# lache/word2vec

Hardware: AMD Instinct MI355X
Metric: trained words/sec, dim=300 SGNS (per-GPU replica, RCCL all-reduce of the replicas' updates for N>1) (higher is better)
Workload: dtype fp32; 1 GPU; sg_ns neg5 d300 w5 subsample 0.0001 min_count 5; synthetic Zipf(s=1) over 1000000 ranks standing in for 1B-Word (configs[2]); 1000-token sentences; vocab_size=740391, global_batch=50000000, parallelism=dp1, hot_rows=-2, private_rows=-1, flush_centers=0, max_waves=0, context_rows=-1, context_flush=0, env_knobs=

## Files before the change

### include/w2v_dev.h

```cpp
#ifndef W2V_DEV_H
#define W2V_DEV_H

#include <stdint.h>

#ifdef __cplusplus
extern "C" {
#endif

#define W2V_OK 0
#define W2V_ERR_ARG 1
#define W2V_ERR_HIP 2
#define W2V_ERR_STATE 3
#define W2V_ERR_UNSUPPORTED 4
#define W2V_ERR_DIVERGED 5
#define W2V_ERR_COMM 6

#define W2V_RNG_PHILOX 0
#define W2V_RNG_REPLAY 1

#define W2V_SCHED_PARALLEL 0
#define W2V_SCHED_SEQUENTIAL 1

#define W2V_UPDATE_PER_PAIR 0
#define W2V_UPDATE_SHARED_NEGATIVES 1
// ... 57 lines not shown
int w2v_dev_upload_corpus(w2v_dev* h, const int32_t* ids, int64_t n_tokens,
                          const int64_t* sent_offsets, int64_t n_sentences,
                          int64_t train_words);
int w2v_dev_share_corpus(w2v_dev* h, w2v_dev* src);
int w2v_dev_upload_replay(w2v_dev* h, const uint32_t* stream, int64_t n,
                          const int64_t* stream_offsets, int64_t n_offsets);

int w2v_dev_set_progress(w2v_dev* h, int64_t current_words);
int w2v_dev_get_progress(w2v_dev* h, int64_t* current_words);
int w2v_dev_set_progress_async(w2v_dev* h, int64_t current_words);
int w2v_dev_set_train_words(w2v_dev* h, int64_t train_words);

int w2v_dev_train_epoch(w2v_dev* h, int32_t epoch, const int64_t* order, w2v_dev_stats* stats);
int w2v_dev_train_epoch_async(w2v_dev* h, int32_t epoch, const int64_t* order_dev);
int w2v_dev_train_sentences_async(w2v_dev* h, int32_t epoch, const int64_t* order_dev, int64_t count);
int w2v_dev_set_order(w2v_dev* h, const int64_t* order, int64_t n);
int w2v_dev_train_slice_async(w2v_dev* h, int32_t epoch, int64_t first, int64_t count);
int w2v_dev_synchronize(w2v_dev* h);
int w2v_dev_read_stats(w2v_dev* h, w2v_dev_stats* stats);
int w2v_dev_reset_stats(w2v_dev* h);

#define W2V_HOT_AUTO (-2)
int w2v_dev_set_hot_rows(w2v_dev* h, int64_t hot_rows);
int w2v_dev_set_hot_auto(w2v_dev* h, float tau_rows, float tau_nodes);
int w2v_dev_hot_tau(w2v_dev* h, float* tau_rows, float* tau_nodes);
int w2v_dev_policy(w2v_dev* h, int64_t* hot_rows, int64_t* hot_nodes, int32_t* private_rows, int32_t* context_rows);
int w2v_dev_flush_policy(w2v_dev* h, int32_t* flush_centers, int32_t* context_flush);
int w2v_dev_row_update_rates(w2v_dev* h, int32_t which, double* out, int64_t n);
int w2v_dev_set_private_rows(w2v_dev* h, int32_t n);
int w2v_dev_set_private_rate(w2v_dev* h, float mu);
int w2v_dev_private_rate_used(w2v_dev* h, float* mu);
int w2v_dev_wave_cap_used(w2v_dev* h, int64_t* waves);
int w2v_dev_deep_used(w2v_dev* h, int32_t* deep);
typedef struct w2v_launch_plan {
  int32_t shared;
  int32_t deep;
  int64_t grid;
  int32_t threads;
  int32_t wpb;
  int64_t lds_bytes;
  int64_t wave_cap;
  int32_t hot_wc;
  int32_t hot_s;
  int64_t hot_atomic;
  int64_t hot_nodes;
  int32_t priv_lo;
  int32_t priv_n;
  int32_t ctx_n;
  float priv_avg;
  int32_t flush_every;
  int32_t ctx_flush_every;
  int32_t nseg;
  int32_t seg_len;
  double private_rate;
  double tau_rows;
  double hs_hot_avg;
  int64_t wide_scratch;
  int64_t n_hot_sc;
  float priv_sc[128];
  float ctx_sc[64];
} w2v_launch_plan;
int w2v_dev_launch_plan(w2v_dev* h, w2v_launch_plan* out, float* hot_sc, int64_t hot_sc_cap);
int w2v_dev_set_replica_count(w2v_dev* h, int32_t n);
int w2v_dev_replica_count(w2v_dev* h, int32_t* n);
int w2v_dev_set_private_sync(w2v_dev* h, int32_t flush_centers, float average_over);
int w2v_dev_set_context_private(w2v_dev* h, int32_t rows, int32_t flush_centers);
// ... 66 lines not shown
```

### word2vec_amd/_native.py

```python
from __future__ import annotations

import ctypes as C
import os
from pathlib import Path

LIB_DIR = Path(__file__).resolve().parent / "lib"
DEV_LIB = LIB_DIR / "libw2v_hip.so"

W2V_OK = 0
W2V_ERR_ARG = 1
W2V_ERR_HIP = 2
W2V_ERR_STATE = 3
W2V_ERR_UNSUPPORTED = 4
W2V_ERR_DIVERGED = 5
W2V_ERR_COMM = 6
W2V_GROUP_ID_BYTES = 128
W2V_GROUP_SUM = 0
W2V_GROUP_AVERAGE = 1
W2V_GROUP_ROW_AVERAGE = 2
W2V_GROUP_ADAPTIVE = 3
W2V_GROUP_SPLIT = 4
W2V_GROUP_SATURATION = 5
W2V_RNG_PHILOX = 0
W2V_RNG_REPLAY = 1
# ... 78 lines not shown
    "w2v_dev_upload_vocab": (C.c_int, [_P, _I64, _P, _P, _P, _P, _P]),
    "w2v_dev_upload_table": (C.c_int, [_P, _P, _I64]),
    "w2v_dev_upload_model": (C.c_int, [_P, _P, _P, _P]),
    "w2v_dev_download_model": (C.c_int, [_P, _P, _P, _P]),
    "w2v_dev_upload_rows": (C.c_int, [_P, _I32, _P, _I64, _P]),
    "w2v_dev_download_rows": (C.c_int, [_P, _I32, _P, _I64, _P]),
    "w2v_dev_bind_model": (C.c_int, [_P, _P, _P, _P, _I64]),
    "w2v_dev_row_pitch": (C.c_int, [_P, C.POINTER(_I64)]),
    "w2v_dev_model_layout": (C.c_int, [_P, C.POINTER(_P), C.POINTER(_P), C.POINTER(_P), C.POINTER(_I64)]),
    "w2v_dev_upload_corpus": (C.c_int, [_P, _P, _I64, _P, _I64, _I64]),
    "w2v_dev_share_corpus": (C.c_int, [_P, _P]),
    "w2v_dev_upload_replay": (C.c_int, [_P, _P, _I64, _P, _I64]),
    "w2v_dev_set_progress": (C.c_int, [_P, _I64]),
    "w2v_dev_get_progress": (C.c_int, [_P, C.POINTER(_I64)]),
    "w2v_dev_set_progress_async": (C.c_int, [_P, _I64]),
    "w2v_dev_set_train_words": (C.c_int, [_P, _I64]),
    "w2v_dev_train_epoch": (C.c_int, [_P, _I32, _P, C.POINTER(DevStats)]),
    "w2v_dev_train_epoch_async": (C.c_int, [_P, _I32, _P]),
    "w2v_dev_train_sentences_async": (C.c_int, [_P, _I32, _P, _I64]),
    "w2v_dev_synchronize": (C.c_int, [_P]),
    "w2v_dev_set_order": (C.c_int, [_P, _P, _I64]),
    "w2v_dev_train_slice_async": (C.c_int, [_P, _I32, _I64, _I64]),
    "w2v_dev_read_stats": (C.c_int, [_P, C.POINTER(DevStats)]),
    "w2v_dev_reset_stats": (C.c_int, [_P]),
    "w2v_dev_set_fixed_alpha": (C.c_int, [_P, _F]),
    "w2v_dev_set_hot_rows": (C.c_int, [_P, _I64]),
    "w2v_dev_set_hot_auto": (C.c_int, [_P, _F, _F]),
    "w2v_dev_policy": (C.c_int, [_P, C.POINTER(_I64), C.POINTER(_I64), C.POINTER(_I32), C.POINTER(_I32)]),
    "w2v_dev_flush_policy": (C.c_int, [_P, C.POINTER(_I32), C.POINTER(_I32)]),
    "w2v_dev_hot_tau": (C.c_int, [_P, C.POINTER(_F), C.POINTER(_F)]),
    "w2v_dev_private_rate_used": (C.c_int, [_P, C.POINTER(_F)]),
    "w2v_dev_wave_cap_used": (C.c_int, [_P, C.POINTER(_I64)]),
    "w2v_dev_deep_used": (C.c_int, [_P, C.POINTER(_I32)]),
    "w2v_dev_launch_plan": (C.c_int, [_P, C.POINTER(LaunchPlan), C.POINTER(C.c_float), _I64]),
    "w2v_dev_set_replica_count": (C.c_int, [_P, _I32]),
    "w2v_dev_model_max_diff": (C.c_int, [_P, _P, C.POINTER(_F)]),
    "w2v_dev_replica_count": (C.c_int, [_P, C.POINTER(_I32)]),
    "w2v_dev_set_private_rows": (C.c_int, [_P, _I32]),
    "w2v_dev_set_private_rate": (C.c_int, [_P, _F]),
    "w2v_dev_set_private_sync": (C.c_int, [_P, _I32, _F]),
    "w2v_dev_set_context_private": (C.c_int, [_P, _I32, _I32]),
    "w2v_dev_set_max_waves": (C.c_int, [_P, _I64]),
    "w2v_dev_set_update": (C.c_int, [_P, _I32]),
    "w2v_dev_apply_rows": (C.c_int, [_P, _P, _P, _I32, _P, _P, _F, _I32]),
    "w2v_dev_score_limits": (C.c_int, [C.POINTER(_I32)] * 3),
    "w2v_dev_set_score_item": (C.c_int, [_P, _I32]),
    "w2v_dev_score": (C.c_int, [_P, _P, _I64, _P, _I64, _U64, _P, _P, C.POINTER(ScoreSummary)]),
    "w2v_group_unique_id": (C.c_int, [_P]),
    "w2v_group_create": (C.c_int, [_P, _I32, _P, _I32, _I32, C.POINTER(_P)]),
    "w2v_group_destroy": (None, [_P]),
    "w2v_group_set_overlap": (C.c_int, [_P, _I32]),
    "w2v_group_set_mode": (C.c_int, [_P, _I32]),
    "w2v_group_set_split": (C.c_int, [_P, _I64, _F]),
    "w2v_group_set_saturation": (C.c_int, [_P, _I64, _F]),
    "w2v_group_row_divisors": (C.c_int, [_P, _I32, C.POINTER(_F), _I64]),
    "w2v_dev_row_update_rates": (C.c_int, [_P, _I32, C.POINTER(C.c_double), _I64]),
    "w2v_group_split_rows": (C.c_int, [_P, C.POINTER(_I64)]),
    "w2v_group_average_async": (C.c_int, [_P]),
    "w2v_group_average_rows_async": (C.c_int, [_P, _I64]),
    "w2v_group_finish": (C.c_int, [_P]),
    "w2v_group_info": (C.c_int, [_P, C.POINTER(_I32), C.POINTER(_I32), C.POINTER(_I32), C.POINTER(_I64)]),
    "w2v_nn_limits": (C.c_int, [C.POINTER(_I32)] * 3),
    "w2v_nn_create": (C.c_int, [_I32, _P, _I64, _I32, C.POINTER(_P)]),
    "w2v_nn_attach": (C.c_int, [_P, _I32, C.POINTER(_P)]),
    "w2v_nn_refresh": (C.c_int, [_P]),
    "w2v_nn_destroy": (None, [_P]),
# ... 73 lines not shown
```

### word2vec_amd/csrc/device/w2v_dev.hip

```cpp
#include <hip/hip_runtime.h>

#include <cstdio>
#include <cstdlib>
#include <algorithm>
#include <cmath>
#include <cstdint>
#include <cstring>
#include <memory>
#include <string>
#include <utility>
#include <vector>

#include "w2v_dev.h"
#include "w2v_dev_internal.hpp"
#include "w2v_kernels.hpp"
#include "w2v_launch.hpp"
#include "w2v_policy.hpp"
#include "w2v_score.hpp"
#include "w2v_shared.hpp"

namespace w2v {

__global__ void expand_table_kernel(const int64_t* bounds, int64_t V, uint32_t* table, int64_t n) {
  const int64_t stride = (int64_t)gridDim.x * blockDim.x;
// ... 76 lines not shown
  w2v::DevBuf<int32_t> points;
  w2v::DevBuf<int64_t> coff;
  int64_t n_codes = 0;
  std::shared_ptr<CorpusBuf> corpus;
  int64_t n_tok = 0, n_sent = 0, train_words = 0;
  int64_t max_len = 0;
  w2v::DevBuf<int64_t> order;
  int64_t n_order = 0;
  w2v::DevBuf<uint32_t> replay;
  w2v::DevBuf<int64_t> replay_off;
  int64_t n_replay_off = 0;
  w2v::DevBuf<unsigned long long> counters;
  w2v::DevBuf<unsigned int> work;
  w2v::DevBuf<float> scratch_f;
  w2v::DevBuf<uint8_t> scratch_codes;
  w2v::DevBuf<int32_t> wide_scratch;
  w2v::DevBuf<float> xfer_f;
  float fixed_alpha = 0.0f;
  int32_t rng = W2V_RNG_PHILOX;
  uint64_t seed = 0;
  int32_t sched = W2V_SCHED_PARALLEL;
  int32_t update = W2V_UPDATE_PER_PAIR;
  int n_cu = 256;
  bool model_ready = false, vocab_ready = false, corpus_ready = false;
  std::vector<float> keep_h;
  std::vector<int32_t> leaf_node;
  std::vector<int32_t> node_parent;
  std::vector<int64_t> tok_count;
  uint64_t data_version = 0;
  uint64_t stats_version = ~0ull;
  w2v::RowStats stats;
  int32_t replicas = 1;
  w2v::LaunchPlan last_plan;
  std::vector<float> hot_sc_h;
  w2v::DevBuf<float> hot_sc_d;
  int32_t score_item = 0;
  w2v::DevBuf<int32_t> score_ids;
  w2v::DevBuf<int64_t> score_soff, score_item_off, score_part_targets, score_targets;
  w2v::DevBuf<double> score_part_ll, score_ll;
  w2v::DevBuf<uint32_t> score_part_nonfinite;
  w2v::DevBuf<unsigned long long> score_ctr;

  ~w2v_dev() {
    (void)hipSetDevice(device);
    if (stream) (void)hipStreamSynchronize(stream);
    if (own_stream && stream) (void)hipStreamDestroy(stream);
  }
  void drop_model() {
    W_own.reset(), C_own.reset(), S_own.reset();
    W = C = S = nullptr;
  }
};

namespace w2v {
int set_error(int code, const std::string& msg) { return fail(code, msg); }
DevInfo dev_info(const w2v_dev* h) { return DevInfo{h->device, h->stream, h->V, h->cfg.word_dim}; }
void set_replicas(w2v_dev* h, int32_t n) { h->replicas = n < 1 ? 1 : n; }
}

static const w2v::RowStats& stats_of(w2v_dev* h) {
  if (h->stats_version != h->data_version) {
    h->stats_version = h->data_version;
    w2v::row_stats(h->stats, h->V, h->tok_count, h->keep_h, h->leaf_node, h->node_parent);
  }
  return h->stats;
}
// ... 8 lines not shown
  for (int64_t c : h->tok_count) N += (double)c;
  const double q = N > 0.0 ? st.kept_tokens / N : 0.0;
  const double win1 = (double)h->cfg.window + 1.0, neg = (double)h->cfg.negative;
  const bool cbow = h->cfg.cbow != 0;
  if (k == 2) {
    if (!st.has_nodes(V)) return false;
    out.resize((size_t)(V - 1));
    for (int64_t j = 0; j < V - 1; ++j) out[(size_t)j] = q * st.node_rate(j, cbow, win1);
    return true;
  }
  out.resize((size_t)V);
  for (int64_t r = 0; r < V; ++r) {
    const double f = st.f[(size_t)r], fk = st.fk[(size_t)r];
    double m;
    if (k == 0) m = cbow ? (neg > 0 ? fk + neg * st.u(r) : 0.0) : fk;
    else m = cbow ? win1 * f : win1 * (f + neg * st.u(r));
    out[(size_t)r] = q * m;
  }
  return true;
}
}

namespace {

using KernelFn = w2v::KernelFn;

const w2v::NvKernels& kernels_for_need(int need) {
  for (const w2v::NvKernels& k : w2v::kNvKernels)
    if (k.nv >= need) return k;
  return *(std::end(w2v::kNvKernels) - 1);
}
int pick_nv(int d) { return kernels_for_need((d + w2v::kWave - 1) / w2v::kWave).nv; }

KernelFn kernel_for(const w2v_dev* h) {
  const bool wd = 2 * h->cfg.window + 1 > w2v::kWave;
  return kernels_for_need(h->nv).pick_train(h->cfg.cbow != 0, h->cfg.hs != 0, h->cfg.negative > 0,
                                            h->rng == W2V_RNG_REPLAY, wd);
}
KernelFn kernel_deep_for(const w2v_dev* h) { return kernels_for_need(h->nv).pick_train_deep(h->cfg.cbow != 0); }
w2v::ApplyFn apply_for(const w2v_dev* h) { return kernels_for_need(h->nv).pick_apply(); }

int set_device(w2v_dev* h) {
  W2V_HIP_TRY(hipSetDevice(h->device));
  return W2V_OK;
}

int install_corpus(w2v_dev* h, std::shared_ptr<CorpusBuf> c, int64_t n_tok, int64_t n_sent, int64_t max_len,
                   int64_t train_words, std::vector<int64_t> hist) {
  w2v::DevBuf<int64_t> order;
  if (int rc = order.alloc((size_t)(n_sent > 0 ? n_sent : 1))) return rc;
  h->corpus = std::move(c);
  h->order = std::move(order);
  h->n_tok = n_tok;
  h->n_sent = n_sent;
  h->n_order = 0;
  h->max_len = max_len;
  h->train_words = train_words;
  h->tok_count = std::move(hist);
  ++h->data_version;
  h->corpus_ready = true;
  return W2V_OK;
}

int init_device(w2v_dev* h) {
  W2V_HIP_TRY(hipSetDevice(h->device));
  W2V_HIP_TRY(hipStreamCreateWithFlags(&h->stream, hipStreamNonBlocking));
  h->own_stream = true;
  if (int rc = h->counters.alloc(8)) return rc;
  W2V_HIP_TRY(hipMemset(h->counters.get(), 0, 8 * sizeof(unsigned long long)));
  if (int rc = h->work.alloc(1)) return rc;
// ... 633 lines not shown
  }
  return W2V_OK;
}

static int launch_train(w2v_dev* h, int32_t epoch, const int64_t* order_dev, int64_t count) {
  w2v::Range range_("w2v launch");
  if (!h->vocab_ready || !h->corpus_ready) return fail(W2V_ERR_STATE, "upload vocab and corpus first");
  if (!h->model_ready) return fail(W2V_ERR_STATE, "upload the model first");
  if (h->cfg.negative > 0 && !h->table.get()) return fail(W2V_ERR_STATE, "no unigram table on the device");
  if (h->rng == W2V_RNG_REPLAY) {
    if (!h->replay.get()) return fail(W2V_ERR_STATE, "replay mode without a replay stream");
    if ((int64_t)(epoch + 1) * h->n_sent > h->n_replay_off)
      return fail(W2V_ERR_ARG, "replay offsets do not cover this epoch");
  }
  if (epoch < 0) return fail(W2V_ERR_ARG, "epoch must be >= 0");
  KernelFn sn_fn = nullptr;
  int sn_waves = 0;
  if (h->update == W2V_UPDATE_SHARED_NEGATIVES) {
    if (int rc = check_shared_negatives(h, true)) return rc;
    const int occ = h->knobs.sn_occ;
    if ((double)h->V * (double)h->pitch * sizeof(float) >= 4294967296.0)
      return fail(W2V_ERR_UNSUPPORTED, "shared negatives: W / C must be < 4 GiB each (32-bit buffer offsets)");
    if (!(sn_fn = w2v::pick_shared_neg(h->pitch, occ, &sn_waves)))
      return fail(W2V_ERR_UNSUPPORTED, "shared negatives: row pitch must be 64 * {1..8,10,12,14,16} floats");
  }
  if (count == 0) return W2V_OK;
  if (set_device(h)) return W2V_ERR_HIP;
  w2v::TrainArgs a{};
  a.W = h->W; a.C = h->C; a.S = h->S;
  a.pitch = h->pitch; a.dim = h->cfg.word_dim;
  a.window = h->cfg.window; a.negative = h->cfg.negative; a.cbow_mean = h->cfg.cbow_mean;
  a.iter = h->cfg.iter; a.init_alpha = h->cfg.init_alpha; a.min_alpha = h->cfg.min_alpha;
  a.train_words = (double)h->train_words;
  a.ids = h->corpus->ids.get(); a.soff = h->corpus->soff.get(); a.order = order_dev; a.n_sent = count; a.n_corpus = h->n_sent;
  a.keep = h->keep.get(); a.table = h->table.get(); a.table_size = h->cfg.table_size;
  a.codes = h->codes.get(); a.points = h->points.get(); a.coff = h->coff.get();
  a.replay = h->replay.get();
  a.replay_off = h->replay_off.get() ? h->replay_off.get() + (int64_t)epoch * h->n_sent : nullptr;
  a.words = h->counters.get();
  a.work = h->work.get();
  a.stats = h->counters.get() + 1;
  a.key0 = (uint32_t)h->seed; a.key1 = (uint32_t)(h->seed >> 32);
  a.epoch = (uint32_t)epoch;
  a.fixed_alpha = h->fixed_alpha;
  a.strict = h->sched == W2V_SCHED_SEQUENTIAL ? 1 : 0;
  W2V_HIP_TRY(hipMemsetAsync(h->work.get(), 0, sizeof(unsigned int), h->stream));
  const KernelFn occ_fn = sn_fn ? sn_fn : kernel_for(h), deep_fn = sn_fn ? sn_fn : kernel_deep_for(h);
  hipError_t occ_err = hipSuccess;
  auto occupancy = [&](w2v::OccKernel k, int threads, int64_t lds) {
    int per_cu = 0;
    const hipError_t e = hipOccupancyMaxActiveBlocksPerMultiprocessor(
        &per_cu, k == w2v::kOccTrainDeep ? deep_fn : occ_fn, threads, (size_t)lds);
    if (e != hipSuccess) occ_err = e;
    return per_cu;
  };
  w2v::LaunchPlan p = w2v::plan_launch(policy_input(h, count, sn_waves), occupancy);
  if (occ_err != hipSuccess)
    return fail(W2V_ERR_HIP, std::string("hipOccupancyMaxActiveBlocksPerMultiprocessor: ") + hipGetErrorString(occ_err));
  if (p.private_rate < 0.0) p.private_rate = h->last_plan.private_rate;
  if (p.tau_rows < 0.0) p.tau_rows = h->last_plan.tau_rows;
  if (p.hs_hot_avg < 0.0) p.hs_hot_avg = h->last_plan.hs_hot_avg;
  a.hot_wc = p.hot_wc; a.hot_s = p.hot_s; a.hot_atomic = p.hot_atomic;
  a.priv_lo = p.priv_lo; a.priv_n = p.priv_n; a.ctx_n = p.ctx_n; a.priv_avg = p.priv_avg;
  a.flush_every = p.flush_every; a.ctx_flush_every = p.ctx_flush_every;
  a.nseg = p.nseg; a.seg_len = p.seg_len;
  std::memcpy(a.priv_sc, p.priv_sc, sizeof(a.priv_sc));
  std::memcpy(a.ctx_sc, p.ctx_sc, sizeof(a.ctx_sc));
  if (!p.shared) {
    if (p.priv_n > 0) a.priv_M = h->cfg.hs ? h->S : (h->cfg.cbow ? h->W : h->C);
    if (p.ctx_n > 0) a.ctx_M = h->C;
  }
  if (int rc = launch_buffers(h, p, a)) return rc;
  const KernelFn fn = p.deep ? deep_fn : occ_fn;
  const dim3 grid((unsigned)p.grid), block((unsigned)p.threads);
  const size_t lds_bytes = (size_t)p.lds_bytes;
  h->last_plan = std::move(p);
  hipLaunchKernelGGL(fn, grid, block, lds_bytes, h->stream, a);
  W2V_HIP_TRY(hipGetLastError());
  return W2V_OK;
}

int w2v_dev_train_epoch(w2v_dev* h, int32_t epoch, const int64_t* order, w2v_dev_stats* st) {
  w2v::Range range_("w2v_dev_train_epoch");
  if (!h) return fail(W2V_ERR_ARG, "null handle");
  w2v_dev_stats before{};
  {
    int rc = w2v_dev_read_stats(h, &before);
    if (rc) return rc;
  }
  const int64_t* od = nullptr;
  if (order) {
    for (int64_t k = 0; k < h->n_sent; ++k)
      if (order[k] < 0 || order[k] >= h->n_sent) return fail(W2V_ERR_ARG, "order entry out of range");
    if (set_device(h)) return W2V_ERR_HIP;
    W2V_HIP_TRY(hipMemcpyAsync(h->order.get(), order, h->n_sent * sizeof(int64_t), hipMemcpyHostToDevice, h->stream));
    od = h->order.get();
    h->n_order = h->n_sent;
  }
  int rc = w2v_dev_train_epoch_async(h, epoch, od);
  if (rc) return rc;
  W2V_HIP_TRY(hipStreamSynchronize(h->stream));
  w2v_dev_stats after{};
  rc = w2v_dev_read_stats(h, &after);
  if (rc) return rc;
  if (st) {
    st->words += after.words - before.words;
    st->centers += after.centers - before.centers;
    st->contexts += after.contexts - before.contexts;
// ... 106 lines not shown
}

int w2v_dev_policy(w2v_dev* h, int64_t* hot_rows, int64_t* hot_nodes, int32_t* private_rows, int32_t* context_rows) {
  if (!h) return fail(W2V_ERR_ARG, "null handle");
  if (hot_rows) *hot_rows = h->last_plan.hot_rows;
  if (hot_nodes) *hot_nodes = h->last_plan.hot_nodes;
  if (private_rows) *private_rows = h->last_plan.priv_n;
  if (context_rows) *context_rows = h->last_plan.ctx_n;
  return W2V_OK;
}

int w2v_dev_hot_tau(w2v_dev* h, float* tau_rows, float* tau_nodes) {
  if (!h) return fail(W2V_ERR_ARG, "null handle");
  if (tau_rows) *tau_rows = (float)h->last_plan.tau_rows;
  if (tau_nodes) *tau_nodes = (float)h->set.hot_tau_nodes;
  return W2V_OK;
}

int w2v_dev_private_rate_used(w2v_dev* h, float* mu) {
  if (!h) return fail(W2V_ERR_ARG, "null handle");
  if (mu) *mu = (float)h->last_plan.private_rate;
  return W2V_OK;
}

int w2v_dev_wave_cap_used(w2v_dev* h, int64_t* waves) {
  if (!h) return fail(W2V_ERR_ARG, "null handle");
  if (waves) *waves = h->last_plan.wave_cap;
  return W2V_OK;
}

int w2v_dev_deep_used(w2v_dev* h, int32_t* deep) {
  if (!h || !deep) return fail(W2V_ERR_ARG, "null argument");
  *deep = h->last_plan.deep ? 1 : 0;
  return W2V_OK;
}

int w2v_dev_launch_plan(w2v_dev* h, w2v_launch_plan* out, float* hot_sc, int64_t hot_sc_cap) {
  if (!h || !out) return fail(W2V_ERR_ARG, "null argument");
  *out = h->last_plan;
  out->n_hot_sc = (int64_t)h->last_plan.hot_sc.size();
  if (hot_sc) std::copy_n(h->last_plan.hot_sc.begin(), std::min(hot_sc_cap, out->n_hot_sc), hot_sc);
  return W2V_OK;
}

int w2v_dev_set_replica_count(w2v_dev* h, int32_t n) {
  if (!h) return fail(W2V_ERR_ARG, "null handle");
  if (n < 1) return fail(W2V_ERR_ARG, "replica count must be >= 1");
  w2v::set_replicas(h, n);
  return W2V_OK;
}

int w2v_dev_replica_count(w2v_dev* h, int32_t* n) {
  if (!h || !n) return fail(W2V_ERR_ARG, "null argument");
  *n = h->replicas;
  return W2V_OK;
}

int w2v_dev_row_update_rates(w2v_dev* h, int32_t which, double* out, int64_t n) {
  if (!h || !out) return fail(W2V_ERR_ARG, "null argument");
  if (which < 0 || which > 2) return fail(W2V_ERR_ARG, "which must be 0 (W), 1 (C) or 2 (synapses1)");
  std::vector<double> rate;
  if (!w2v::row_update_rates(h, which, rate)) return fail(W2V_ERR_STATE, "no vocab / corpus statistics uploaded");
  if (n != (int64_t)rate.size()) return fail(W2V_ERR_ARG, "n must be the matrix's row count");
  std::copy(rate.begin(), rate.end(), out);
  return W2V_OK;
}
// ... 175 lines not shown
```

### word2vec_amd/csrc/device/w2v_inst.hip

```cpp
#include "w2v_kernels.hpp"
#include "w2v_launch.hpp"

#ifndef W2V_NV
#error "build with -DW2V_NV=<floats per lane>"
#endif

#define W2V_CAT2(a, b) a##b
#define W2V_CAT(a, b) W2V_CAT2(a, b)

namespace w2v {

constexpr int kMaxT = W2V_NV <= 16 ? 8 : 4;

KernelFn W2V_CAT(pick_train_nv, W2V_NV)(bool cbow, bool hs, bool ns, bool replay, bool wide) {
#define W2V_K(CB, H, N, R, WD) &train_epoch_kernel<W2V_NV, kMaxT, CB, H, N, R, WD>
#define W2V_KR(CB, H, N, WD) (replay ? W2V_K(CB, H, N, true, WD) : W2V_K(CB, H, N, false, WD))
#define W2V_KW(H, N) (wide ? W2V_KR(true, H, N, true) : W2V_KR(true, H, N, false))
  if (cbow) {
    if (hs && ns) return W2V_KW(true, true);
    if (hs) return W2V_KW(true, false);
    return W2V_KW(false, true);
  }
  if (hs && ns) return W2V_KR(false, true, true, false);
  if (hs) return W2V_KR(false, true, false, false);
  return W2V_KR(false, false, true, false);
#undef W2V_KW
#undef W2V_KR
#undef W2V_K
}

KernelFn W2V_CAT(pick_train_deep_nv, W2V_NV)(bool cbow) {
  constexpr int M = kDeepMaxT<W2V_NV>;
  return cbow ? &train_epoch_deep_kernel<W2V_NV, M, true, true, false, false, false>
              : &train_epoch_deep_kernel<W2V_NV, M, false, true, false, false, false>;
}

ApplyFn W2V_CAT(pick_apply_nv, W2V_NV)() { return &apply_rows_kernel<W2V_NV>; }

}
```

### word2vec_amd/csrc/device/w2v_kernels.hpp

```cpp
#pragma once
#include <hip/hip_runtime.h>
#include <stdint.h>

#include "w2v_limits.hpp"
#include "w2v_philox.hpp"
#include "w2v_rows.hpp"
#include "w2v_wave.hpp"

namespace w2v {


struct TrainArgs {
  float* W;
  float* C;
  float* S;
  int64_t pitch;
  int32_t dim;
  int32_t window;
  int32_t negative;
  int32_t cbow_mean;
  int32_t iter;
  float init_alpha;
  float min_alpha;
  double train_words;
// ... 5 lines not shown
  const float* keep;
  const uint32_t* table;
  int64_t table_size;
  const uint8_t* codes;
  const int32_t* points;
  const int64_t* coff;
  const uint32_t* replay;
  const int64_t* replay_off;
  unsigned long long* words;
  unsigned int* work;
  unsigned long long* stats;
  uint32_t key0, key1, epoch;
  float fixed_alpha;
  int32_t hot_wc;
  int32_t hot_s;
  const float* hot_sc;
  int32_t strict;
  const float* priv_M;
  int32_t priv_lo;
  int32_t priv_n;
  float priv_avg;
  int32_t flush_every;
  const float* ctx_M;
  int32_t ctx_n;
  int32_t ctx_flush_every;
  int32_t* wide_ids;
  int64_t wide_stride;
  int64_t item0;
  int64_t hot_atomic;
  int32_t nseg;
  int32_t seg_len;
  float priv_sc[128];
  float ctx_sc[64];
};

struct Counters {
  unsigned long long centers = 0, contexts = 0, targets = 0, draws = 0, sentences = 0;
#ifdef W2V_PP_PROF
  unsigned long long t = 0, acc[8] = {0, 0, 0, 0, 0, 0, 0, 0};
  __device__ void stamp(int k) {
    const unsigned long long now = __builtin_amdgcn_s_memtime();
    acc[k] += now - t;
    t = now;
  }
#else
  __device__ void stamp(int) {}
#endif
};

constexpr int kNonFinite = 5;

__device__ __forceinline__ void report_counters(const TrainArgs& a, const Counters& cnt) {
  atomicAdd(&a.stats[0], cnt.centers);
  atomicAdd(&a.stats[1], cnt.contexts);
  atomicAdd(&a.stats[2], cnt.targets);
  atomicAdd(&a.stats[3], cnt.draws);
  atomicAdd(&a.stats[4], cnt.sentences);
}

__device__ __forceinline__ float scheduled_alpha(const TrainArgs& a) {
  const unsigned long long cw = __hip_atomic_load(a.words, __ATOMIC_RELAXED, __HIP_MEMORY_SCOPE_AGENT);
  const float al = (float)(a.init_alpha * (1.0 - 1.0 / a.iter * (double)cw / a.train_words));
  return (a.min_alpha < al) ? al : a.min_alpha;
}


struct PrivRows {
  float* delta = nullptr;
  unsigned long long* dirty = nullptr;
  unsigned* lock = nullptr;
  float* M = nullptr;
  int lo = 0;
  int n = 0;
  bool ctx = false;
  __device__ bool has(int row) const { return (unsigned)(row - lo) < (unsigned)n; }
};

template <int NV>
__device__ __forceinline__ PrivRows out_rows(const TrainArgs& a, float* lds) {
  PrivRows p;
  if (lds == nullptr || a.priv_n == 0) return p;
  p.dirty = reinterpret_cast<unsigned long long*>(lds + kLdsDirtyOut);
  p.lock = reinterpret_cast<unsigned*>(lds) + kLdsLockOut;
  p.delta = lds + kLdsHeaderWords;
  p.M = const_cast<float*>(a.priv_M);
  p.lo = a.priv_lo;
  p.n = a.priv_n;
  return p;
}

template <int NV>
__device__ __forceinline__ PrivRows ctx_rows(const TrainArgs& a, float* lds) {
  PrivRows p;
  if (lds == nullptr || a.ctx_n == 0) return p;
  p.dirty = reinterpret_cast<unsigned long long*>(lds + kLdsDirtyCtx);
  p.lock = reinterpret_cast<unsigned*>(lds) + kLdsLockCtx;
// ... 632 lines not shown
  }
}

template <int NV, int MAXT, bool CBOW, bool HS, bool NS, bool REPLAY, bool WIDE>
__device__ __forceinline__ void train_epoch(const TrainArgs& a) {
  extern __shared__ float w2v_lds[];
  const int lane = lane_id();
  float* lds = (a.priv_n + a.ctx_n) > 0 ? w2v_lds : nullptr;
  if (lds) {
    const int64_t words = kLdsHeaderWords + (int64_t)(a.priv_n + a.ctx_n) * (NV * kWave);
    for (int64_t k = threadIdx.x; k < words; k += blockDim.x) lds[k] = 0.0f;
    __syncthreads();
  }
  Counters cnt;
#ifdef W2V_PP_PROF
  cnt.t = __builtin_amdgcn_s_memtime();
#endif
  float alpha = a.init_alpha;
  bool first = true;
  const uint32_t wmax = (uint32_t)(a.window < 1 ? 1 : a.window);
  const uint32_t nseg = (uint32_t)(a.nseg > 1 ? a.nseg : 1);
  const int64_t n_items = a.n_sent * (int64_t)nseg;
  for (;;) {
    uint32_t kk = 0;
    if (lane == 0) kk = atomicAdd(a.work, 1u);
    kk = (uint32_t)uniform_i((int)kk);
    if ((int64_t)kk >= n_items) break;
    const uint32_t k = kk / nseg, seg = kk - k * nseg;
    const int64_t s = a.order ? a.order[k] : (int64_t)k;
    if (s < 0 || s >= a.n_corpus) continue;
    if (a.fixed_alpha > 0.0f) {
      alpha = a.fixed_alpha;
    } else if (first || (k % 10u) == 0u) {
      alpha = scheduled_alpha(a);
      first = false;
    }
    const int64_t base = a.soff[s];
    const int len = (int)(a.soff[s + 1] - base);
    const int32_t* sent = a.ids + base;
    const uint32_t* rp = nullptr;
    if (REPLAY) {
      rp = a.replay + a.replay_off[s];
      for (int i = 0; i < len; ++i) {
        const int c = sent[i];
        const float u = __int_as_float((int)rp[0]);
        ++rp;
        if (a.keep[c] < u) continue;
        const int rw = (int)rp[0];
        ++rp;
        center<NV, MAXT, CBOW, HS, NS, REPLAY, WIDE>(a, lds, sent, len, i, c, rw, (uint32_t)s, alpha, rp, cnt, lane);
      }
    } else {
      const int seg_lo = nseg > 1 ? min(len, (int)seg * a.seg_len) : 0;
      const int seg_hi = nseg > 1 ? min(len, seg_lo + a.seg_len) : len;
      for (int i0 = seg_lo; i0 < seg_hi; i0 += kWave) {
        const int ii = i0 + lane;
        const bool in = ii < seg_hi;
        const int c_l = in ? sent[ii] : 0;
        const float p_l = in ? a.keep[c_l] : 0.f;
        float u_l;
        int rw_l;
        subsample_draw(a, (uint32_t)s, (uint32_t)ii, wmax, u_l, rw_l);
        unsigned long long kept = ballot(in && !(p_l < u_l));
        while (kept) {
          const int b = __builtin_ctzll(kept);
          kept &= kept - 1;
          const int c = readlane_i(c_l, b), rw = readlane_i(rw_l, b);
          center<NV, MAXT, CBOW, HS, NS, REPLAY, WIDE>(a, lds, sent, len, i0 + b, c, rw, (uint32_t)s, alpha, rp,
                                                        cnt, lane);
        }
      }
    }
    if (REPLAY || nseg == 1) {
      if (lane == 0) atomicAdd(a.words, (unsigned long long)len);
      cnt.sentences += 1;
    } else {
      const int seg_lo = min(len, (int)seg * a.seg_len), seg_hi = min(len, seg_lo + a.seg_len);
      if (lane == 0 && seg_hi > seg_lo) atomicAdd(a.words, (unsigned long long)(seg_hi - seg_lo));
      cnt.sentences += (seg == 0) ? 1 : 0;
    }
  }
  flush_private<NV>(a, out_rows<NV>(a, lds), lane);
  flush_private<NV>(a, ctx_rows<NV>(a, lds), lane);
#ifdef W2V_PP_PROF
  cnt.stamp(0);
  if (lane == 0 && (threadIdx.x / kWave) % 4 == 0 && (blockIdx.x == 0 || blockIdx.x == gridDim.x / 2))
    printf("PPPROF block %u wave %d centers %llu: %llu %llu %llu %llu %llu %llu %llu %llu\n", blockIdx.x,
           (int)(threadIdx.x / kWave), cnt.centers, cnt.acc[0], cnt.acc[1], cnt.acc[2], cnt.acc[3], cnt.acc[4],
           cnt.acc[5], cnt.acc[6], cnt.acc[7]);
#endif
  if (lane == 0) report_counters(a, cnt);
}

template <int NV, int MAXT, bool CBOW, bool HS, bool NS, bool REPLAY, bool WIDE>
__global__ __launch_bounds__(kMaxBlock<NV>, kMinWaves<NV>) void train_epoch_kernel(TrainArgs a) {
  train_epoch<NV, MAXT, CBOW, HS, NS, REPLAY, WIDE>(a);
}

template <int NV>
constexpr int kDeepMaxT = NV <= 2 ? 32 : NV <= 4 ? 24 : NV <= 6 ? 16 : NV <= 16 ? 8 : 4;
template <int NV, int MAXT, bool CBOW, bool HS, bool NS, bool REPLAY, bool WIDE>
__global__ __launch_bounds__(kDeepBlock, 2) void train_epoch_deep_kernel(TrainArgs a) {
  train_epoch<NV, MAXT, CBOW, HS, NS, REPLAY, WIDE>(a);
}

template <int NV>
__global__ __launch_bounds__(64) void apply_rows_kernel(float* M, int64_t pitch, int d, const float* x_in,
                                                        float* grad_io, const uint8_t* codes, int n, float alpha,
                                                        int hs_form) {
  const int lane = lane_id();
  float x[NV], g[NV];
#pragma unroll
// ... 21 lines not shown
```

### word2vec_amd/csrc/device/w2v_launch.hpp

```cpp
#pragma once
#include <stdint.h>

namespace w2v {

struct TrainArgs;
using KernelFn = void (*)(TrainArgs);
using ApplyFn = void (*)(float*, int64_t, int, const float*, float*, const uint8_t*, int, float, int);

#define W2V_FOR_EACH_NV(X) X(1) X(2) X(3) X(4) X(5) X(6) X(8) X(12) X(16) X(24) X(32)

#define W2V_DECLARE_NV(N)                                            \
  KernelFn pick_train_nv##N(bool cbow, bool hs, bool ns, bool replay, bool wide); \
  KernelFn pick_train_deep_nv##N(bool cbow); \
  ApplyFn pick_apply_nv##N();
W2V_FOR_EACH_NV(W2V_DECLARE_NV)
#undef W2V_DECLARE_NV

struct NvKernels {
  int nv;
  KernelFn (*pick_train)(bool cbow, bool hs, bool ns, bool replay, bool wide);
  KernelFn (*pick_train_deep)(bool cbow);
  ApplyFn (*pick_apply)();
};
#define W2V_NV_ROW(N) {N, pick_train_nv##N, pick_train_deep_nv##N, pick_apply_nv##N},
inline const NvKernels kNvKernels[] = {W2V_FOR_EACH_NV(W2V_NV_ROW)};
#undef W2V_NV_ROW

KernelFn pick_shared_neg(int64_t pitch, int occ, int* waves);

}
```

### word2vec_amd/csrc/device/w2v_rows.hpp

```cpp
#pragma once
#include <hip/hip_runtime.h>
#include <stdint.h>

#include "w2v_limits.hpp"

namespace w2v {

template <int NV>
__device__ __forceinline__ void load_row(const float* M, int64_t row, int64_t pitch, int lane, bool fresh,
                                         float (&r)[NV]) {
  const float* p = M + row * pitch + lane;
  if (fresh) {
#pragma unroll
    for (int v = 0; v < NV; ++v) r[v] = __hip_atomic_load(p + kWave * v, __ATOMIC_RELAXED, __HIP_MEMORY_SCOPE_AGENT);
  } else {
#pragma unroll
    for (int v = 0; v < NV; ++v) r[v] = p[kWave * v];
  }
}

template <int NV>
__device__ __forceinline__ void store_row(float* M, int64_t row, int64_t pitch, int lane, const float (&r)[NV]) {
  float* p = M + row * pitch + lane;
#pragma unroll
  for (int v = 0; v < NV; ++v) p[kWave * v] = r[v];
}

template <int NV>
constexpr int kFullVecs = NV <= 6 ? NV - 1 : NV == 8 ? 6 : NV == 12 ? 8 : NV == 16 ? 12 : NV == 24 ? 16 : 24;

template <int NV>
__device__ __forceinline__ void atomic_add_row(float* M, int64_t row, int64_t pitch, int d, int lane,
                                               const float (&delta)[NV]) {
  float* p = M + row * pitch + lane;
#pragma unroll
  for (int v = 0; v < NV; ++v)
    if (v < kFullVecs<NV> || lane + kWave * v < d)
      (void)__hip_atomic_fetch_add(p + kWave * v, delta[v], __ATOMIC_RELAXED, __HIP_MEMORY_SCOPE_AGENT);
}

template <int NV>
__device__ __forceinline__ void add_to_row(float* M, int64_t row, bool hot, int64_t pitch, int d, int lane,
                                           const float (&delta)[NV]) {
  if (hot) {
    atomic_add_row<NV>(M, row, pitch, d, lane, delta);
  } else {
    float cur[NV];
    load_row<NV>(M, row, pitch, lane, false, cur);
#pragma unroll
    for (int v = 0; v < NV; ++v) cur[v] += delta[v];
    store_row<NV>(M, row, pitch, lane, cur);
  }
}

}
```

### word2vec_amd/device.py

```python
from __future__ import annotations

import ctypes as C
from dataclasses import dataclass

import numpy as np

from . import _native as N


def _ptr(a: np.ndarray | None):
    if a is None:
        return None
    assert a.flags["C_CONTIGUOUS"], "arrays passed to the C-ABI must be C-contiguous"
    return a.ctypes.data_as(C.c_void_p)


@dataclass
class Config:

    word_dim: int = 200
    window: int = 5
    negative: int = 0
    hs: bool = True
    cbow: bool = True
# ... 166 lines not shown
    def synchronize(self):
        self._chk(self.lib.w2v_dev_synchronize(self.h), "w2v_dev_synchronize")

    def read_stats(self) -> dict:
        st = N.DevStats()
        self._chk(self.lib.w2v_dev_read_stats(self.h, C.byref(st)), "w2v_dev_read_stats")
        return st.as_dict()

    def knobs(self) -> str:
        return self.lib.w2v_dev_knobs(self.h).decode()

    def reset_stats(self):
        self._chk(self.lib.w2v_dev_reset_stats(self.h), "w2v_dev_reset_stats")

    def set_hot_rows(self, hot_rows: int):
        self._chk(self.lib.w2v_dev_set_hot_rows(self.h, int(hot_rows)), "w2v_dev_set_hot_rows")

    def set_hot_auto(self, tau_rows: float = 0.0, tau_nodes: float = 1.0):
        self._chk(self.lib.w2v_dev_set_hot_auto(self.h, float(tau_rows), float(tau_nodes)), "w2v_dev_set_hot_auto")

    def policy(self) -> dict:
        r, n, p, c = C.c_int64(), C.c_int64(), C.c_int32(), C.c_int32()
        self._chk(self.lib.w2v_dev_policy(self.h, C.byref(r), C.byref(n), C.byref(p), C.byref(c)), "w2v_dev_policy")
        f, cf = C.c_int32(), C.c_int32()
        self._chk(self.lib.w2v_dev_flush_policy(self.h, C.byref(f), C.byref(cf)), "w2v_dev_flush_policy")
        tr, tn = C.c_float(), C.c_float()
        self._chk(self.lib.w2v_dev_hot_tau(self.h, C.byref(tr), C.byref(tn)), "w2v_dev_hot_tau")
        mu = C.c_float()
        self._chk(self.lib.w2v_dev_private_rate_used(self.h, C.byref(mu)), "w2v_dev_private_rate_used")
        wc = C.c_int64()
        self._chk(self.lib.w2v_dev_wave_cap_used(self.h, C.byref(wc)), "w2v_dev_wave_cap_used")
        dp = C.c_int32()
        self._chk(self.lib.w2v_dev_deep_used(self.h, C.byref(dp)), "w2v_dev_deep_used")
        return {"hot_rows": r.value, "hot_nodes": n.value, "private_rows": p.value, "context_rows": c.value,
                "flush_centers": f.value, "context_flush": cf.value, "hot_tau_rows": tr.value,
                "private_rate": round(mu.value, 4), "wave_cap": wc.value, "deep": dp.value}

    def launch_plan(self) -> dict:
        p = N.LaunchPlan()
        self._chk(self.lib.w2v_dev_launch_plan(self.h, C.byref(p), None, 0), "w2v_dev_launch_plan")
        hot = np.zeros(p.n_hot_sc, np.float32)
        if hot.size:
            buf = hot.ctypes.data_as(C.POINTER(C.c_float))
            self._chk(self.lib.w2v_dev_launch_plan(self.h, C.byref(p), buf, hot.size), "w2v_dev_launch_plan")
        skip = ("n_hot_sc", "priv_sc", "ctx_sc")
        out = {k: getattr(p, k) for k, _ in p._fields_ if k not in skip}
        out.update(priv_sc=np.array(p.priv_sc, np.float32), ctx_sc=np.array(p.ctx_sc, np.float32), hot_sc=hot)
        return out

    def set_private_rows(self, n: int):
        self._chk(self.lib.w2v_dev_set_private_rows(self.h, int(n)), "w2v_dev_set_private_rows")

    def set_private_rate(self, mu: float):
        self._chk(self.lib.w2v_dev_set_private_rate(self.h, float(mu)), "w2v_dev_set_private_rate")

    def set_private_sync(self, flush_centers: int = 0, average_over: float = 8.0):
        self._chk(self.lib.w2v_dev_set_private_sync(self.h, int(flush_centers), float(average_over)),
                  "w2v_dev_set_private_sync")

    def set_context_private(self, rows: int = -1, flush_centers: int = 0):
        self._chk(self.lib.w2v_dev_set_context_private(self.h, int(rows), int(flush_centers)),
                  "w2v_dev_set_context_private")

    def row_update_rates(self, which: int, rows: int) -> np.ndarray:
        out = np.empty(rows, np.float64)
        self._chk(self.lib.w2v_dev_row_update_rates(self.h, int(which), out.ctypes.data_as(C.POINTER(C.c_double)),
                                                    int(rows)), "w2v_dev_row_update_rates")
        return out

# ... 40 lines not shown
```

Measured before the change: 106.3 million words/s.

## Specialize SG-NS kernel batch width and use scalar row base addressing

Adds a dedicated skip-gram negative-sampling kernel instantiation whose target batch equals negative+1 when negative is small, instead of the generic maximum batch. Row loads, stores and atomics now compute a wave-uniform base address via readfirstlane plus a per-lane 32-bit offset, so addressing can use scalar registers. The alpha schedule precomputes the inverse iteration count and the sentence counter is kept wave-uniform. Together these aim to cut vector register pressure and address arithmetic in the hot loop. The risk is changed occupancy or codegen behaviour for other NV sizes, and a new ABI query is added for the chosen batch.

```diff
diff --git a/include/w2v_dev.h b/include/w2v_dev.h
--- a/include/w2v_dev.h
+++ b/include/w2v_dev.h
@@ -113,6 +113,7 @@
 int w2v_dev_private_rate_used(w2v_dev* h, float* mu);
 int w2v_dev_wave_cap_used(w2v_dev* h, int64_t* waves);
 int w2v_dev_deep_used(w2v_dev* h, int32_t* deep);
+int w2v_dev_ns_batch_used(w2v_dev* h, int32_t* rows);
 typedef struct w2v_launch_plan {
   int32_t shared;
   int32_t deep;
diff --git a/word2vec_amd/_native.py b/word2vec_amd/_native.py
--- a/word2vec_amd/_native.py
+++ b/word2vec_amd/_native.py
@@ -134,6 +134,7 @@
     "w2v_dev_private_rate_used": (C.c_int, [_P, C.POINTER(_F)]),
     "w2v_dev_wave_cap_used": (C.c_int, [_P, C.POINTER(_I64)]),
     "w2v_dev_deep_used": (C.c_int, [_P, C.POINTER(_I32)]),
+    "w2v_dev_ns_batch_used": (C.c_int, [_P, C.POINTER(_I32)]),
     "w2v_dev_launch_plan": (C.c_int, [_P, C.POINTER(LaunchPlan), C.POINTER(C.c_float), _I64]),
     "w2v_dev_set_replica_count": (C.c_int, [_P, _I32]),
     "w2v_dev_model_max_diff": (C.c_int, [_P, _P, C.POINTER(_F)]),
diff --git a/word2vec_amd/csrc/device/w2v_dev.hip b/word2vec_amd/csrc/device/w2v_dev.hip
--- a/word2vec_amd/csrc/device/w2v_dev.hip
+++ b/word2vec_amd/csrc/device/w2v_dev.hip
@@ -132,6 +132,7 @@
   w2v::RowStats stats;
   int32_t replicas = 1;
   w2v::LaunchPlan last_plan;
+  int last_ns_batch = 0;
   std::vector<float> hot_sc_h;
   w2v::DevBuf<float> hot_sc_d;
   int32_t score_item = 0;
@@ -206,10 +207,10 @@
 }
 int pick_nv(int d) { return kernels_for_need((d + w2v::kWave - 1) / w2v::kWave).nv; }
 
-KernelFn kernel_for(const w2v_dev* h) {
+KernelFn kernel_for(const w2v_dev* h, int* ns_batch) {
   const bool wd = 2 * h->cfg.window + 1 > w2v::kWave;
   return kernels_for_need(h->nv).pick_train(h->cfg.cbow != 0, h->cfg.hs != 0, h->cfg.negative > 0,
-                                            h->rng == W2V_RNG_REPLAY, wd);
+                                            h->rng == W2V_RNG_REPLAY, wd, h->cfg.negative, ns_batch);
 }
 KernelFn kernel_deep_for(const w2v_dev* h) { return kernels_for_need(h->nv).pick_train_deep(h->cfg.cbow != 0); }
 w2v::ApplyFn apply_for(const w2v_dev* h) { return kernels_for_need(h->nv).pick_apply(); }
@@ -909,6 +910,7 @@
   a.window = h->cfg.window; a.negative = h->cfg.negative; a.cbow_mean = h->cfg.cbow_mean;
   a.iter = h->cfg.iter; a.init_alpha = h->cfg.init_alpha; a.min_alpha = h->cfg.min_alpha;
   a.train_words = (double)h->train_words;
+  a.inv_iter = 1.0 / h->cfg.iter; a.init_alpha_d = (double)h->cfg.init_alpha;
   a.ids = h->corpus->ids.get(); a.soff = h->corpus->soff.get(); a.order = order_dev; a.n_sent = count; a.n_corpus = h->n_sent;
   a.keep = h->keep.get(); a.table = h->table.get(); a.table_size = h->cfg.table_size;
   a.codes = h->codes.get(); a.points = h->points.get(); a.coff = h->coff.get();
@@ -922,7 +924,8 @@
   a.fixed_alpha = h->fixed_alpha;
   a.strict = h->sched == W2V_SCHED_SEQUENTIAL ? 1 : 0;
   W2V_HIP_TRY(hipMemsetAsync(h->work.get(), 0, sizeof(unsigned int), h->stream));
-  const KernelFn occ_fn = sn_fn ? sn_fn : kernel_for(h), deep_fn = sn_fn ? sn_fn : kernel_deep_for(h);
+  int ns_batch = 0;
+  const KernelFn occ_fn = sn_fn ? sn_fn : kernel_for(h, &ns_batch), deep_fn = sn_fn ? sn_fn : kernel_deep_for(h);
   hipError_t occ_err = hipSuccess;
   auto occupancy = [&](w2v::OccKernel k, int threads, int64_t lds) {
     int per_cu = 0;
@@ -951,6 +954,7 @@
   const KernelFn fn = p.deep ? deep_fn : occ_fn;
   const dim3 grid((unsigned)p.grid), block((unsigned)p.threads);
   const size_t lds_bytes = (size_t)p.lds_bytes;
+  h->last_ns_batch = (fn == occ_fn && h->cfg.negative > 0) ? ns_batch : 0;
   h->last_plan = std::move(p);
   hipLaunchKernelGGL(fn, grid, block, lds_bytes, h->stream, a);
   W2V_HIP_TRY(hipGetLastError());
@@ -1123,6 +1127,12 @@
 int w2v_dev_deep_used(w2v_dev* h, int32_t* deep) {
   if (!h || !deep) return fail(W2V_ERR_ARG, "null argument");
   *deep = h->last_plan.deep ? 1 : 0;
+  return W2V_OK;
+}
+
+int w2v_dev_ns_batch_used(w2v_dev* h, int32_t* rows) {
+  if (!h || !rows) return fail(W2V_ERR_ARG, "null argument");
+  *rows = h->last_ns_batch;
   return W2V_OK;
 }
 
diff --git a/word2vec_amd/csrc/device/w2v_inst.hip b/word2vec_amd/csrc/device/w2v_inst.hip
--- a/word2vec_amd/csrc/device/w2v_inst.hip
+++ b/word2vec_amd/csrc/device/w2v_inst.hip
@@ -12,7 +12,17 @@
 
 constexpr int kMaxT = W2V_NV <= 16 ? 8 : 4;
 
-KernelFn W2V_CAT(pick_train_nv, W2V_NV)(bool cbow, bool hs, bool ns, bool replay, bool wide) {
+constexpr int kNsSmall = 5;
+constexpr int kSgNsT = W2V_NV > 16 ? kMaxT : kNsSmall + 1;
+
+KernelFn W2V_CAT(pick_train_nv, W2V_NV)(bool cbow, bool hs, bool ns, bool replay, bool wide, int negative,
+                                        int* ns_batch) {
+  *ns_batch = kMaxT;
+  if (!cbow && !hs && ns && negative <= kNsSmall) {
+    *ns_batch = kSgNsT;
+    return replay ? &train_epoch_kernel<W2V_NV, kSgNsT, false, false, true, true, false>
+                  : &train_epoch_kernel<W2V_NV, kSgNsT, false, false, true, false, false>;
+  }
 #define W2V_K(CB, H, N, R, WD) &train_epoch_kernel<W2V_NV, kMaxT, CB, H, N, R, WD>
 #define W2V_KR(CB, H, N, WD) (replay ? W2V_K(CB, H, N, true, WD) : W2V_K(CB, H, N, false, WD))
 #define W2V_KW(H, N) (wide ? W2V_KR(true, H, N, true) : W2V_KR(true, H, N, false))
diff --git a/word2vec_amd/csrc/device/w2v_kernels.hpp b/word2vec_amd/csrc/device/w2v_kernels.hpp
--- a/word2vec_amd/csrc/device/w2v_kernels.hpp
+++ b/word2vec_amd/csrc/device/w2v_kernels.hpp
@@ -61,6 +61,8 @@
   int32_t seg_len;
   float priv_sc[128];
   float ctx_sc[64];
+  double inv_iter;
+  double init_alpha_d;
 };
 
 struct Counters {
@@ -87,10 +89,13 @@
   atomicAdd(&a.stats[4], cnt.sentences);
 }
 
+__device__ __forceinline__ float scheduled_alpha(const TrainArgs& a, double inv_iter, double init_alpha) {
+  const unsigned long long cw = __hip_atomic_load(a.words, __ATOMIC_RELAXED, __HIP_MEMORY_SCOPE_AGENT);
+  const float al = (float)(init_alpha * (1.0 - inv_iter * (double)cw / a.train_words));
+  return (a.min_alpha < al) ? al : a.min_alpha;
+}
 __device__ __forceinline__ float scheduled_alpha(const TrainArgs& a) {
-  const unsigned long long cw = __hip_atomic_load(a.words, __ATOMIC_RELAXED, __HIP_MEMORY_SCOPE_AGENT);
-  const float al = (float)(a.init_alpha * (1.0 - 1.0 / a.iter * (double)cw / a.train_words));
-  return (a.min_alpha < al) ? al : a.min_alpha;
+  return scheduled_alpha(a, 1.0 / a.iter, (double)a.init_alpha);
 }
 
 
@@ -789,7 +794,7 @@
     if (a.fixed_alpha > 0.0f) {
       alpha = a.fixed_alpha;
     } else if (first || (k % 10u) == 0u) {
-      alpha = scheduled_alpha(a);
+      alpha = scheduled_alpha(a, a.inv_iter, a.init_alpha_d);
       first = false;
     }
     const int64_t base = a.soff[s];
@@ -830,11 +835,11 @@
     }
     if (REPLAY || nseg == 1) {
       if (lane == 0) atomicAdd(a.words, (unsigned long long)len);
-      cnt.sentences += 1;
+      cnt.sentences = uniform_u64(cnt.sentences + 1);
     } else {
       const int seg_lo = min(len, (int)seg * a.seg_len), seg_hi = min(len, seg_lo + a.seg_len);
       if (lane == 0 && seg_hi > seg_lo) atomicAdd(a.words, (unsigned long long)(seg_hi - seg_lo));
-      cnt.sentences += (seg == 0) ? 1 : 0;
+      cnt.sentences = uniform_u64(cnt.sentences + ((seg == 0) ? 1 : 0));
     }
   }
   flush_private<NV>(a, out_rows<NV>(a, lds), lane);
diff --git a/word2vec_amd/csrc/device/w2v_launch.hpp b/word2vec_amd/csrc/device/w2v_launch.hpp
--- a/word2vec_amd/csrc/device/w2v_launch.hpp
+++ b/word2vec_amd/csrc/device/w2v_launch.hpp
@@ -10,7 +10,7 @@
 #define W2V_FOR_EACH_NV(X) X(1) X(2) X(3) X(4) X(5) X(6) X(8) X(12) X(16) X(24) X(32)
 
 #define W2V_DECLARE_NV(N)                                            \
-  KernelFn pick_train_nv##N(bool cbow, bool hs, bool ns, bool replay, bool wide); \
+  KernelFn pick_train_nv##N(bool cbow, bool hs, bool ns, bool replay, bool wide, int negative, int* ns_batch); \
   KernelFn pick_train_deep_nv##N(bool cbow); \
   ApplyFn pick_apply_nv##N();
 W2V_FOR_EACH_NV(W2V_DECLARE_NV)
@@ -18,7 +18,7 @@
 
 struct NvKernels {
   int nv;
-  KernelFn (*pick_train)(bool cbow, bool hs, bool ns, bool replay, bool wide);
+  KernelFn (*pick_train)(bool cbow, bool hs, bool ns, bool replay, bool wide, int negative, int* ns_batch);
   KernelFn (*pick_train_deep)(bool cbow);
   ApplyFn (*pick_apply)();
 };
diff --git a/word2vec_amd/csrc/device/w2v_rows.hpp b/word2vec_amd/csrc/device/w2v_rows.hpp
--- a/word2vec_amd/csrc/device/w2v_rows.hpp
+++ b/word2vec_amd/csrc/device/w2v_rows.hpp
@@ -7,23 +7,44 @@
 namespace w2v {
 
 template <int NV>
+constexpr bool kScalarBase = NV != 8 && NV != 24;
+using GlobalRow = __attribute__((address_space(1))) float*;
+template <int NV>
+__device__ __forceinline__ GlobalRow row_base(const float* M, int64_t row, int64_t pitch, int lane, uint32_t& o) {
+  if constexpr (!kScalarBase<NV>) {
+    o = 0u;
+    return (GlobalRow)reinterpret_cast<uint64_t>(M + row * pitch + lane);
+  } else {
+    const uint64_t p = reinterpret_cast<uint64_t>(M + row * pitch);
+    const uint32_t lo = (uint32_t)__builtin_amdgcn_readfirstlane((int)(uint32_t)p);
+    const uint32_t hi = (uint32_t)__builtin_amdgcn_readfirstlane((int)(uint32_t)(p >> 32));
+    o = (uint32_t)lane;
+    return (GlobalRow)(((uint64_t)hi << 32) | lo);
+  }
+}
+
+template <int NV>
 __device__ __forceinline__ void load_row(const float* M, int64_t row, int64_t pitch, int lane, bool fresh,
                                          float (&r)[NV]) {
-  const float* p = M + row * pitch + lane;
+  uint32_t o;
   if (fresh) {
+    const GlobalRow p = row_base<NV>(M, row, pitch, lane, o);
 #pragma unroll
-    for (int v = 0; v < NV; ++v) r[v] = __hip_atomic_load(p + kWave * v, __ATOMIC_RELAXED, __HIP_MEMORY_SCOPE_AGENT);
+    for (int v = 0; v < NV; ++v)
+      r[v] = __hip_atomic_load((p + kWave * v) + o, __ATOMIC_RELAXED, __HIP_MEMORY_SCOPE_AGENT);
   } else {
+    const GlobalRow p = row_base<NV>(M, row, pitch, lane, o);
 #pragma unroll
-    for (int v = 0; v < NV; ++v) r[v] = p[kWave * v];
+    for (int v = 0; v < NV; ++v) r[v] = (p + kWave * v)[o];
   }
 }
 
 template <int NV>
 __device__ __forceinline__ void store_row(float* M, int64_t row, int64_t pitch, int lane, const float (&r)[NV]) {
-  float* p = M + row * pitch + lane;
+  uint32_t o;
+  const GlobalRow p = row_base<NV>(M, row, pitch, lane, o);
 #pragma unroll
-  for (int v = 0; v < NV; ++v) p[kWave * v] = r[v];
+  for (int v = 0; v < NV; ++v) (p + kWave * v)[o] = r[v];
 }
 
 template <int NV>
@@ -32,11 +53,12 @@
 template <int NV>
 __device__ __forceinline__ void atomic_add_row(float* M, int64_t row, int64_t pitch, int d, int lane,
                                                const float (&delta)[NV]) {
-  float* p = M + row * pitch + lane;
+  uint32_t o;
+  const GlobalRow p = row_base<NV>(M, row, pitch, lane, o);
 #pragma unroll
   for (int v = 0; v < NV; ++v)
     if (v < kFullVecs<NV> || lane + kWave * v < d)
-      (void)__hip_atomic_fetch_add(p + kWave * v, delta[v], __ATOMIC_RELAXED, __HIP_MEMORY_SCOPE_AGENT);
+      (void)__hip_atomic_fetch_add((p + kWave * v) + o, delta[v], __ATOMIC_RELAXED, __HIP_MEMORY_SCOPE_AGENT);
 }
 
 template <int NV>
diff --git a/word2vec_amd/device.py b/word2vec_amd/device.py
--- a/word2vec_amd/device.py
+++ b/word2vec_amd/device.py
@@ -222,9 +222,12 @@
         self._chk(self.lib.w2v_dev_wave_cap_used(self.h, C.byref(wc)), "w2v_dev_wave_cap_used")
         dp = C.c_int32()
         self._chk(self.lib.w2v_dev_deep_used(self.h, C.byref(dp)), "w2v_dev_deep_used")
+        nb = C.c_int32()
+        self._chk(self.lib.w2v_dev_ns_batch_used(self.h, C.byref(nb)), "w2v_dev_ns_batch_used")
         return {"hot_rows": r.value, "hot_nodes": n.value, "private_rows": p.value, "context_rows": c.value,
                 "flush_centers": f.value, "context_flush": cf.value, "hot_tau_rows": tr.value,
-                "private_rate": round(mu.value, 4), "wave_cap": wc.value, "deep": dp.value}
+                "private_rate": round(mu.value, 4), "wave_cap": wc.value, "deep": dp.value,
+                "ns_batch": nb.value}
 
     def launch_plan(self) -> dict:
         p = N.LaunchPlan()
```

After: 105.4 million words/s (median of 2 runs). Within noise of the previous version (-0.8%).
